# submarine0418/underwater_image_enhancement

Measured on AMD Instinct MI355X. Metric: megapixels/sec enhanced, higher is better.
Workload: dtype f32/f64

## Files before the change

underwater_image_enhancement_amd/csrc/api.hip:

```cpp
#include <cstdarg>
#include <cstdio>
#include <cstring>

#include "common.h"

#include <cstdlib>

namespace uwie {

static thread_local char g_err[512] = "";
static thread_local uwie_ctx *g_ctx = nullptr;
static const Tuning g_default_tuning{};

const Tuning &tune() { return g_ctx ? g_ctx->tune : g_default_tuning; }
uwie_ctx *current_ctx() { return g_ctx; }

void set_error(const char *fmt, ...)
{
    va_list ap;
    va_start(ap, fmt);
    vsnprintf(g_err, sizeof g_err, fmt, ap);
    va_end(ap);
}

// ... 29 lines not shown
        return UWIE_E_HIP;                                                    \
    }

struct KnobName { const char *name; int Tuning::*field; };
const KnobName kKnobs[] = {{"gf_split", &Tuning::gf_split}, {"gf_bands", &Tuning::gf_bands},
                           {"select_generic", &Tuning::select_generic}, {"restore_store", &Tuning::restore_store},
                           {"lin_predict3", &Tuning::lin_predict3}, {"lin_cap", &Tuning::lin_cap},
                           {"lin_no_predict", &Tuning::lin_no_predict}, {"q_hist", &Tuning::q_hist}, {"lin_predict_shift", &Tuning::lin_predict_shift},
                           {"streams", &Tuning::streams}, {"canny_prepass", &Tuning::canny_prepass},
                           {"canny_fault_inject", &Tuning::canny_fault_inject}, {"rank_sweep", &Tuning::rank_sweep},
                           {"gf_fuse", &Tuning::gf_fuse}, {"entry_fuse", &Tuning::entry_fuse}};

void tuning_from_env(Tuning *t)
{
    for (const KnobName &k : kKnobs) {
        char var[64] = "UWIE_";
        size_t n = 5;
        for (const char *c = k.name; *c && n + 1 < sizeof var; ++c) var[n++] = (char)(*c >= 'a' && *c <= 'z' ? *c - 32 : *c);
        var[n] = 0;
        if (const char *e = getenv(var)) t->*(k.field) = atoi(e);
    }
}

bool shape_ok(int B, int H, int W)
{
    if (B < 1 || H < 1 || W < 1) return false;
    const long long npx = (long long)H * W;
    return npx < (1ll << 30) && (long long)B * npx < (1ll << 40);
}

#define UWIE_CHECK_SHAPE(B, H, W) UWIE_REQUIRE(shape_ok(B, H, W), "batch/H/W out of range")
#define UWIE_CHECK_WS(need)                                                                           \
    do {                                                                                              \
        if ((need) > 0 && (!d_workspace || workspace_bytes < (need))) {                               \
            set_error("workspace too small: need %zu bytes, got %zu", (size_t)(need), workspace_bytes); \
            return UWIE_E_WORKSPACE;                                                                  \
        }                                                                                             \
    } while (0)
#define UWIE_TRY(call)            \
    do {                          \
        int _rc = (call);         \
        if (_rc != UWIE_OK) return _rc; \
    } while (0)

struct Pipe {
    int32_t *kind;
    float *A;
    float *pct;
    float *F;
    double *F64;
    double *pct64;
    uint8_t *gray;
    float *t0;
    double *t;
    void *scratch;
    size_t scratch_bytes;
    bool planes;
    uint32_t *qpart;
    int32_t *guess;
};

size_t max5(size_t a, size_t b, size_t c, size_t d, size_t e)
{
    size_t m = a;
    if (b > m) m = b;
    if (c > m) m = c;
    if (d > m) m = d;
    if (e > m) m = e;
    return m;
}

bool dehazes(const uwie_params *p)
{
    if (p->surface == UWIE_SURFACE_SIX) return p->strategy >= 1 && p->strategy <= 3;
    return p->strategy >= UWIE_DICT_STRONG_DEHAZING && p->strategy <= UWIE_DICT_LIGHT_ENHANCEMENT;
}

GuidedRequest u8_guided(const uwie_params *p)
{
    const bool six = p->surface == UWIE_SURFACE_SIX;
    GuidedRequest r{p->gf_ksize, p->gf_eps, p->gf_exact != 0};
    r.fx = six && p->inter_dtype == UWIE_INTER_FX32;
    r.f32_ok = six && p->inter_dtype == UWIE_INTER_F32T && !tune().select_generic;
    r.t0_from_frame = true;
    return r;
}

Pipe carve_pipe(Carver &c, Shape s, const uwie_params *p)
{
    Pipe P{};
    const size_t n = (size_t)s.B * s.npx();
    P.kind = c.take<int32_t>(s.B);
    P.A = c.take<float>((size_t)s.B * 3);
    P.pct = c.take<float>((size_t)s.B * 3 * kMaxPct);
    P.guess = c.take<int32_t>(s.B);
    const bool dz = !p || dehazes(p);
    const bool dict_dz = p && p->surface == UWIE_SURFACE_DICT && dz;
    if (dict_dz) {
        P.F64 = c.take<double>(n * 3);
        P.pct64 = c.take<double>((size_t)s.B * 3 * kMaxPct);
    } else if (!p || (p->surface == UWIE_SURFACE_SIX && dz && (p->strategy == 3 || tune().restore_store || tune().select_generic))) {
        P.F = c.take<float>(n * 3);
    }
    const int tx = p ? p->tiles_x : 8, ty = p ? p->tiles_y : 8;
    const bool gf_planes = dz && (!p || plan_guided(s, u8_guided(p)).planes);
    if (dz) {
        P.gray = c.take<uint8_t>(n);
        if (gf_planes) P.t0 = c.take<float>(n);
        P.t = c.take<double>(n);
    }
    P.scratch_bytes = max5(cast_ws_bytes(s), dz ? airlight_ws_bytes(s) : 0, gf_planes ? guided_ws_bytes(s) : 0,
                           select_ws_bytes(s), clahe_ws_bytes(s, tx > 0 ? tx : 8, ty > 0 ? ty : 8));
    const size_t cw = codes_ws_bytes(s, tx > 0 ? tx : 8, ty > 0 ? ty : 8);
    if (cw > P.scratch_bytes) P.scratch_bytes = cw;
    if (dz && !gf_planes && P.scratch_bytes < n * sizeof(float)) P.scratch_bytes = n * sizeof(float);
    size_t qoff = 0;
    if (dz && p && p->surface == UWIE_SURFACE_SIX && p->cast_correct && p->forced_cast < 0 && entry_fuse_takes(s, p->min_size)) {
        qoff = (std::max(cast_ws_bytes(s), airlight_ws_bytes(s)) + 255) & ~size_t(255);
        if (P.scratch_bytes < qoff + quad_part_bytes(s)) P.scratch_bytes = qoff + quad_part_bytes(s);
    }
    P.scratch = c.take<char>(P.scratch_bytes);
    P.planes = gf_planes;
    if (dz && !gf_planes) P.t0 = static_cast<float *>(P.scratch);
    if (qoff && P.scratch) P.qpart = reinterpret_cast<uint32_t *>(static_cast<char *>(P.scratch) + qoff);
    return P;
}

uwie_params merged_params(const uwie_params *ps, int n, Shape s)
{
    uwie_params m = ps[0];
    m.surface = UWIE_SURFACE_SIX;
    m.strategy = 2;
    for (int i = 0; i < n; ++i) {
        if (ps[i].surface == UWIE_SURFACE_SIX && ps[i].strategy == 3) m.strategy = 3;
        if (ps[i].tiles_x > m.tiles_x) m.tiles_x = ps[i].tiles_x;
        if (ps[i].tiles_y > m.tiles_y) m.tiles_y = ps[i].tiles_y;
        if (ps[i].surface == UWIE_SURFACE_SIX && ps[i].strategy <= 3 && plan_guided(s, u8_guided(&ps[i])).planes) m.gf_exact = 1;
    }
    return m;
}

int stage_guided(const Pipe &P, Shape s, const uwie_params *p, const FuseT0Args &frame, hipStream_t st, int *t_is_f32 = nullptr)
{
    const GuidedPlan g = plan_guided(s, u8_guided(p));
    UWIE_REQUIRE(!g.planes || (P.planes && P.t0 != P.scratch), "guided filter: the workspace layout has no planes for the exact-order filter");
    if (g.t0) UWIE_TRY(launch_trans_init(frame.rgb, frame.kind, frame.A, s, frame.omega, frame.norm_eps, frame.pre_clip, P.t0, st));
    UWIE_TRY(launch_guided_plan(g, s, P.gray, P.t0, P.t, P.scratch, st, &frame));
    if (t_is_f32) *t_is_f32 = g.t_f32;
    return UWIE_OK;
}

int stretch_f32(const float *img, float *out, Shape s, double lo, double hi, float eps, float *pct, void *ws, hipStream_t st)
{
    const double q[2] = {lo, hi};
    UWIE_TRY(launch_percentiles(img, 0, s, q, 2, pct, ws, st));
    return launch_stretch_apply_f32(img, pct, 2, 0, 1, eps, out, s, st);
}

bool quad_from_cast(const uwie_params *p, const Pipe &P) { return P.qpart && p->forced_cast < 0 && p->cast_correct; }

int six_cast(uwie_ctx *ctx, const uint8_t *d_in, Shape s, const uwie_params *p, const Pipe &P, const int32_t **kind,
             hipStream_t st, bool then_airlight = false)
{
    *kind = nullptr;
    if (p->forced_cast >= 0) {
        UWIE_TRY(launch_set_kind(P.kind, s.B, p->forced_cast, st));
        *kind = P.kind;
    } else if (p->cast_correct) {
        const EntryFuse ef{P.qpart, tune().entry_fuse == 2 ? nullptr : P.gray, P.guess, p->gray_shift};
        UWIE_TRY(launch_cast_classify(ctx, d_in, s, P.kind, nullptr, P.scratch, st, then_airlight && quad_from_cast(p, P) ? &ef : nullptr));
        *kind = P.kind;
    }
    return UWIE_OK;
}

int six_airlight(uwie_ctx *ctx, const uint8_t *d_in, const int32_t *kind, Shape s, const uwie_params *p, const Pipe &P,
                 hipStream_t st, bool after_cast = false)
{
    const bool fused = after_cast && quad_from_cast(p, P);
    return launch_airlight(ctx, d_in, kind, P.gray, s, p->min_size, P.A, nullptr, P.scratch, st,
                           fused && tune().entry_fuse != 2 ? 0 : p->gray_shift, fused ? P.qpart : nullptr);
}

int six_dehaze_tail(uwie_ctx *ctx, const uint8_t *d_in, const int32_t *kind, Shape s, const uwie_params *p, const Pipe &P,
                    uint8_t *d_out_u8, float *d_out_f32, hipStream_t st)
{
    const float eps = 1e-6f;
    const int k = p->strategy;
    int t_is_f32 = 0;
    UWIE_TRY(stage_guided(P, s, p, FuseT0Args{d_in, kind, P.A, (float)p->omega, 1e-6f, 1}, st, &t_is_f32));
    SelectPlan plan;
    const double q[4] = {p->L_low, p->L_high, p->wb_percentile, 100 - p->wb_percentile};
    const RestoreSrc src{d_in, kind, P.A, P.t, t_is_f32};
    bool recompute = false;
    if (tune().select_generic) {
        UWIE_TRY(select_begin<float>(s, q, k == 3 ? 4 : 2, P.scratch, st, &plan));
        UWIE_TRY(launch_restore_planar_hist(d_in, kind, P.A, P.t, s, P.F, plan.ghist, st, false, nullptr, t_is_f32));
        UWIE_TRY(select_run(plan, P.F, 1, s, true, st));
    } else {
        recompute = k != 3 && !tune().restore_store;
// ... 1503 lines not shown
```

underwater_image_enhancement_amd/csrc/common.h:

```cpp
#pragma once
#include <hip/hip_runtime.h>
#include <stddef.h>
#include <stdint.h>

#include "../../include/uwie.h"

namespace uwie {

void set_error(const char *fmt, ...);
#define UWIE_HIP_CHECK(expr)                                                            \
    do {                                                                                \
        hipError_t _e = (expr);                                                         \
        if (_e != hipSuccess) {                                                         \
            ::uwie::set_error("%s failed: %s (%s:%d)", #expr, hipGetErrorString(_e), __FILE__, __LINE__); \
            return UWIE_E_HIP;                                                          \
        }                                                                               \
    } while (0)
#define UWIE_LAUNCH_CHECK() UWIE_HIP_CHECK(hipGetLastError())
#define UWIE_REQUIRE(cond, msg)                 \
    do {                                        \
        if (!(cond)) {                          \
            ::uwie::set_error("%s", msg);       \
            return UWIE_E_INVALID;              \
        }                                       \
// ... 159 lines not shown
uint32_t *canny_strong_flags(void *ws, Shape s);
int launch_make_full_regions(Region *d_regions, Shape s, hipStream_t st);

int launch_region_stats(const uint8_t *d_in, const int32_t *d_kind, const Region *d_regs, int nreg, int max_rows,
                        int max_cols, Shape s, float *csum, int maxChunks, float *tot, float *mean, float *vtot,
                        hipStream_t st);
int launch_frame_hist(const uint8_t *d_in, Shape s, uint32_t *d_hist, hipStream_t st);
size_t features_ws_bytes(Shape s);
int launch_features_u8(const uint8_t *d_in, Shape s, float *d_out, void *ws, hipStream_t st);

size_t quality_ws_bytes(Shape s);
int launch_quality_scores(uwie_ctx *ctx, const uint8_t *d_u8, const float *d_f32, Shape s, int gray_shift,
                          const double *weights8, double *d_scores, void *ws, hipStream_t st);

bool feature_extractor_has_dct(int H, int W);
int feature_extractor_count(int H, int W);
size_t feature_extractor_ws_bytes(Shape s);
int launch_feature_extractor(uwie_ctx *ctx, const uint8_t *d_u8, const float *d_f32, Shape s, int gray_shift, double *d_out,
                             void *ws, hipStream_t st);

int launch_resize_rgb(const uwie_frame_desc *d_desc, int B, int oh, int ow, const uint8_t *d_flips, uint8_t *d_u8, float *d_f32,
                      float *d_norm, const float *mean3, const float *std3, uint32_t *d_status, hipStream_t st);

struct ClsNode {
    double thr;
    int32_t left, right, feat, miss;
};
struct ClsModel {
    int kind, F, C, T, K, S;
    double lr, gamma;
    const double *mean, *scale;
    const int32_t *tree_off;
    const ClsNode *nodes;
    const double *value;
    const double *init;
    const double *svT;
    const double *coef;
    const double *rho;
    const double *prob_a, *prob_b;
    const int32_t *sv_start;
};
int classify_model_check(const uwie_model_desc *d);
size_t classify_blob_bytes(const uwie_model_desc *d);
ClsModel classify_pack(const uwie_model_desc *d, void *host_blob, const void *dev_blob);
int launch_classify(const ClsModel &m, const double *d_rows, int B, int32_t *d_label, double *d_proba, uint32_t *d_status,
                    hipStream_t st);

int launch_pick_best(const double *d_scores, int n, Shape s, const uint8_t *d_all, int32_t *d_best, uint8_t *d_out, hipStream_t st);

size_t guided_ws_bytes(Shape s);
size_t box_ws_bytes(Shape s);
int launch_trans_init(const uint8_t *d_in, const int32_t *d_kind, const float *d_A, Shape s, float omega, float norm_eps,
                      int pre_clip, float *d_t0, hipStream_t st);
int launch_box_filter_f64(const double *d_src, double *d_dst, Shape s, int k, void *ws, hipStream_t st);
int launch_guided(const uint8_t *d_gray, const float *d_t0, Shape s, int k, double eps, double *d_t, void *ws,
                  hipStream_t st);
int launch_guided_p64(const uint8_t *d_gray, const double *d_t0, Shape s, int k, double eps, double *d_t, void *ws, hipStream_t st);

enum GuidedRoute {
    GF_EXACT,
    GF_FAST,
    GF_PIPE,
    GF_SPLIT,
    GF_FUSED,
};
struct GuidedRequest {
    int k;
    double eps;
    bool exact = false;
    bool fx = false;
    bool f32_ok = false;
    bool t0_from_frame = false;
    bool t0_f64 = false;
};
struct GuidedPlan {
    GuidedRoute route;
    int k;
    double eps;
    bool t_f32;
    bool ring_fx;
    bool t0_f64;
    bool t0;
    bool planes;
    int TH;
    int iy0, band, nb, rows;
    int pipe_bands;
};
GuidedPlan plan_guided(Shape s, const GuidedRequest &r);
struct FuseT0Args {
    const uint8_t *rgb;
    const int32_t *kind;
    const float *A;
    float omega, norm_eps;
    int pre_clip;
};
int launch_guided_plan(const GuidedPlan &g, Shape s, const uint8_t *d_gray, const void *d_t0, double *d_t, void *ws, hipStream_t st,
                       const FuseT0Args *frame = nullptr);
int guided_fast_th(Shape s, int k);
int launch_guided_fast(const uint8_t *d_gray, const float *d_t0, Shape s, int k, int TH, double eps, double *d_t, hipStream_t st);

constexpr int kMaxPct = 4;
size_t select_ws_bytes(Shape s);
template <typename V>
int launch_percentiles(const V *d_vals, int planar, Shape s, const double *q_percent, int nq, V *d_out, void *ws, hipStream_t st);
int launch_widen_f32(const float *d_in, double *d_out, size_t n, hipStream_t st);

constexpr int kSelGroupStride = 2 * kMaxPct * 2048;
constexpr int kSelOsStride = 2 * kMaxPct;
struct LinState;
struct SelectPlan {
    void *state;
    uint32_t *ghist;
    void *os;
    double t[kMaxPct];
    int nq;
    bool is64;
    LinState *lin;
    void *lists;
    uint32_t *flags;
    uint32_t cap;
    bool predicted;
    uint32_t ranks[2 * kMaxPct];
    template <typename V>
    V *lists_as() const { return static_cast<V *>(lists); }
};
constexpr int kLinBins = 2050;
__host__ __device__ inline uint32_t lin_digit(float x)
{
    if (!(x > 0.0f)) return 0;
    if (x >= 1.0f) return kLinBins - 1;
    const uint32_t d = (uint32_t)(x * 2048.0f);
    return 1 + (d > 2047u ? 2047u : d);
}
__host__ __device__ inline uint32_t lin_digit(double x)
{
    if (!(x > 0.0)) return 0;
    if (x >= 1.0) return kLinBins - 1;
    const uint32_t d = (uint32_t)(x * 2048.0);
    return 1 + (d > 2047u ? 2047u : d);
}
constexpr int kLinLists = 2 * kMaxPct;
constexpr uint32_t kLinNoWin = 0x80000000u;
struct LinState {
    uint32_t rr[2 * kMaxPct];
    uint32_t qbin[2 * kMaxPct];
    uint32_t gid[2 * kMaxPct];
    uint32_t gbin[2 * kMaxPct];
// ... 130 lines not shown
```

underwater_image_enhancement_amd/csrc/k_guided.hip:

```cpp
#include "common.h"
#include "devutil.h"
#include "guided_wave.h"

namespace uwie {

namespace {

typedef double2 __attribute__((aligned(8))) gdouble2_a8;
typedef float4 __attribute__((aligned(4))) gfloat4_a4;
typedef uint32_t __attribute__((aligned(1))) gu32_a1;
typedef double gd2v __attribute__((ext_vector_type(2), aligned(8)));
__device__ __forceinline__ void st_d2(double *p, double v0, double v1) { __builtin_nontemporal_store(gd2v{v0, v1}, reinterpret_cast<gd2v *>(p)); }
__device__ __forceinline__ void st_d1(double *p, double v) { __builtin_nontemporal_store(v, p); }
__device__ __forceinline__ double ld_d1(const double *p) { return __builtin_nontemporal_load(p); }

struct SrcPlanes1 {
    const double *p;
    int H, W;
    static constexpr const char *kName = "k_box_rows_lane<SrcPlanes1>";
    static constexpr int NP = 1;
    static constexpr int CH = 16;
    struct Raw {
        double v;
    };
// ... 631 lines not shown
    const uint8_t *img = in + (size_t)b * npx * 3;
    const bool aligned = (npx & 3) == 0;
    for (int i = threadIdx.x; i < 768; i += 256) {
        const int c = i >> 8;
        nrm[c][i & 255] = px_val(i & 255, px_atten(k, c)) / (A[b * 3 + c] + norm_eps);
    }
    __syncthreads();
    float *trow = t0 + (size_t)b * npx;
    auto t_of = [&](const Px4 &v, int i) {
        const float dark = fminf(fminf(nrm[0][v.r[i]], nrm[1][v.g[i]]), nrm[2][v.b[i]]);
        float t = 1.0f - omega * dark;
        if (pre_clip) t = fminf(fmaxf(t, 0.1f), 1.0f);
        return t;
    };
#ifndef UWIE_TI_PREFETCH
#define UWIE_TI_PREFETCH 1
#endif
    if (UWIE_TI_PREFETCH && aligned && npx >= 4) {
        const int stride = gridDim.x * 1024, plast = npx - 4;
        int p = (blockIdx.x * 256 + threadIdx.x) * 4;
        auto ld3 = [&](int q) { return *reinterpret_cast<const uint3 *>(img + (size_t)q * 3); };
        uint3 nx = ld3(min(p, plast));
        for (; p < npx; p += stride) {
            const uint3 w = nx;
            nx = ld3(min(p + stride, plast));
            Px4 v;
            v.r[0] = w.x & 255; v.g[0] = (w.x >> 8) & 255; v.b[0] = (w.x >> 16) & 255;
            v.r[1] = w.x >> 24; v.g[1] = w.y & 255; v.b[1] = (w.y >> 8) & 255;
            v.r[2] = (w.y >> 16) & 255; v.g[2] = w.y >> 24; v.b[2] = w.z & 255;
            v.r[3] = (w.z >> 8) & 255; v.g[3] = (w.z >> 16) & 255; v.b[3] = w.z >> 24;
            *reinterpret_cast<float4 *>(trow + p) = make_float4(t_of(v, 0), t_of(v, 1), t_of(v, 2), t_of(v, 3));
        }
        return;
    }
    for (int p = (blockIdx.x * 256 + threadIdx.x) * 4; p < npx; p += gridDim.x * 1024) {
        const int n = min(4, npx - p);
        const Px4 v = load_px4(img + (size_t)p * 3, n, aligned);
        float o[4];
#pragma unroll
        for (int i = 0; i < 4; ++i) {
            const float dark = fminf(fminf(nrm[0][v.r[i]], nrm[1][v.g[i]]), nrm[2][v.b[i]]);
            float t = 1.0f - omega * dark;
            if (pre_clip) t = fminf(fmaxf(t, 0.1f), 1.0f);
            o[i] = t;
        }
        if (aligned && n == 4) {
            *reinterpret_cast<float4 *>(trow + p) = make_float4(o[0], o[1], o[2], o[3]);
        } else {
            for (int i = 0; i < n; ++i) trow[p + i] = o[i];
        }
    }
}

}

int launch_trans_init(const uint8_t *d_in, const int32_t *d_kind, const float *d_A, Shape s, float omega, float norm_eps,
                      int pre_clip, float *d_t0, hipStream_t st)
{
#ifndef UWIE_TI_BLOCKS
#define UWIE_TI_BLOCKS 16384
#endif
    int blocks = grid_for((s.npx() + 3) / 4, 4096);
    {
        int want = cdiv(UWIE_TI_BLOCKS, s.B);
        want = want < 32 ? 32 : want;
        if (blocks > want) blocks = want;
    }
    UWIE_LAUNCH(k_trans_init, dim3(blocks, s.B), dim3(256), 0, st, d_in, d_kind, d_A, (int)s.npx(), omega,
                       norm_eps, pre_clip, d_t0);
    UWIE_LAUNCH_CHECK();
    return UWIE_OK;
}

size_t box_ws_bytes(Shape s)
{
    Carver c(nullptr);
    c.take<double>((size_t)s.B * s.npx());
    return c.total();
}

int launch_box_filter_f64(const double *d_src, double *d_dst, Shape s, int k, void *ws, hipStream_t st)
{
    Carver c(ws);
    const size_t n = (size_t)s.B * s.npx();
    double *rs = c.take<double>(n);
    launch_rows_planes(d_src, nullptr, s, rs, n, k, st);
    UWIE_LAUNCH_CHECK();
    launch_cols(rs, n, EpiStore1{d_dst}, s, k, st);
    UWIE_LAUNCH_CHECK();
    return UWIE_OK;
}

size_t guided_ws_bytes(Shape s)
{
    Carver c(nullptr);
    c.take<double>((size_t)s.B * s.npx() * 6);
    return c.total();
}

template <class TP>
static int launch_guided_t(const uint8_t *d_gray, const TP *d_t0, Shape s, int k, double eps, double *d_t, void *ws, hipStream_t st)
{
    Carver c(ws);
    const size_t n = (size_t)s.B * s.npx();
    double *rs = c.take<double>(n * 6);
    double *pa = rs + 4 * n, *pb = rs + 5 * n;
// ... 34 lines not shown
```

underwater_image_enhancement_amd/csrc/k_guided_pipe.hip:

```cpp
#include "common.h"
#include "devutil.h"
#include "guided_wave.h"

#include <algorithm>
#include <cmath>
#include <type_traits>
#include <utility>

namespace uwie {

namespace {

#define UWIE_TRY_RC(call)               \
    do {                                \
        const int _rc = (call);         \
        if (_rc != UWIE_OK) return _rc; \
    } while (0)

#ifndef UWIE_GF_MINBAND
#define UWIE_GF_MINBAND 32
#endif
constexpr int kPipeSlots = 128;
struct PipeGeom {
    int H, W, band;
// ... 493 lines not shown
        } else rest.template swap_at<S - 1>(a0, a1, gg);
    }
    template <int S>
    __device__ __forceinline__ void set_at(uint32_t a0, uint32_t a1, uint32_t gg)
    {
        if constexpr (S == 0) {
            t0 = a0; t1 = a1;
            if constexpr (G) g = gg;
        } else rest.template set_at<S - 1>(a0, a1, gg);
    }
};
template <bool G>
struct RawRing<0, G> {
    template <int S> __device__ __forceinline__ void swap_at(uint32_t &, uint32_t &, uint32_t &) {}
    template <int S> __device__ __forceinline__ void set_at(uint32_t, uint32_t, uint32_t) {}
};

#ifndef SPLIT_QUAD
#define SPLIT_QUAD 1
#endif
#ifndef SPLIT_MUL24
#define SPLIT_MUL24 1
#endif
__device__ __forceinline__ double dpp_next(double v)
{
    const int lo = __builtin_amdgcn_update_dpp(0, __double2loint(v), 0x130, 0xf, 0xf, true);
    const int hi = __builtin_amdgcn_update_dpp(0, __double2hiint(v), 0x130, 0xf, 0xf, true);
    return __hiloint2double(hi, lo);
}
__device__ __forceinline__ uint32_t dpp_next(uint32_t v)
{
    return (uint32_t)__builtin_amdgcn_update_dpp(0, (int)v, 0x130, 0xf, 0xf, true);
}
__device__ __forceinline__ double2 q_add(double2 a, double2 b) { return make_double2(a.x + b.x, a.y + b.y); }
__device__ __forceinline__ double2 q_sub(double2 a, double2 b) { return make_double2(a.x - b.x, a.y - b.y); }
__device__ __forceinline__ double2 q_next(double2 v) { return make_double2(dpp_next(v.x), dpp_next(v.y)); }
__device__ __forceinline__ uint2 q_add(uint2 a, uint2 b) { return make_uint2(a.x + b.x, a.y + b.y); }
__device__ __forceinline__ uint2 q_sub(uint2 a, uint2 b) { return make_uint2(a.x - b.x, a.y - b.y); }
__device__ __forceinline__ uint2 q_next(uint2 v) { return make_uint2(dpp_next(v.x), dpp_next(v.y)); }

template <int K>
struct SplitCfg {
    static constexpr bool RAWREG = K <= 16;
    static constexpr int NB = K % 3 == 0 ? 3 : K > 16 ? 2 : K % 5 == 0 ? 5 : 2;
    static constexpr int AR = K > 16 ? 3 : 0;
    static constexpr bool STAGE_FIRST = AR > 0;
    static constexpr int pad_bytes = 16 * (PipeCfg<K>::M + 1) > 128 ? 16 * (PipeCfg<K>::M + 1) : 128;
    static constexpr int s2_bytes = STAGE_FIRST ? 2048 : 2048 + pad_bytes;
    static constexpr int ring_lds_bytes = (K - AR) * (PipeCfg<K>::NL + 1) * 16;
    static_assert(!STAGE_FIRST || ring_lds_bytes >= pad_bytes, "the look-ahead must stay inside the allocation");
    static constexpr int lds_bytes = ring_lds_bytes + PipeCfg<K>::s1_doubles * 8 + s2_bytes;
};

__device__ __forceinline__ uint32_t fuse_t0_bits(const float *tab, uint32_t r, uint32_t g, uint32_t b, float omega, int pre_clip)
{
    const float dark = fminf(fminf(tab[r], tab[256 + g]), tab[512 + b]);
    float t = __fsub_rn(1.0f, __fmul_rn(omega, dark));
    if (pre_clip) t = fminf(fmaxf(t, 0.1f), 1.0f);
    return __float_as_uint(t);
}

template <int K, bool EDGE, typename TOut, bool FUSE = false>
__device__ __forceinline__ void split_body(const uint8_t *__restrict__ gray, const float *__restrict__ t0, TOut *__restrict__ tout,
                                           const SplitGeom &g, const PipeConsts &cs, char *lds, int3 bid, int lane_in = -1,
                                           const float *tab = nullptr, float omega = 0.0f, int pre_clip = 0)
{
    using C = PipeCfg<K>;
    constexpr int a = C::a, Lb = C::Lb, NV = C::NV, RC = K, NL = C::NL, M = C::M, SW = C::SW;
    constexpr int NB = SplitCfg<K>::NB;
    static_assert(RC % NB == 0, "the ring period must be a multiple of the row buffers");
    constexpr bool RAWREG = SplitCfg<K>::RAWREG;
    constexpr int NLp = NL + 1, EB = 16;
    constexpr int AR = SplitCfg<K>::AR;
    constexpr int ring_bytes = SplitCfg<K>::ring_lds_bytes;
    constexpr uint32_t stage_base = SplitCfg<K>::STAGE_FIRST ? 0u : (uint32_t)ring_bytes;
    constexpr uint32_t ring_base = SplitCfg<K>::STAGE_FIRST ? 3072u + 2048u : 0u;
    constexpr double K2 = (double)(K * K);
    const int lane = lane_in >= 0 ? lane_in : (int)threadIdx.x;
    const int H = g.H, W = g.W;
    const int x_lo = bid.x * NV;
    const int y_lo = g.y0 + bid.y * g.band;
    const int r_lo = y_lo - a;
    const size_t img = (size_t)bid.z * H * W;
    const uint32_t npx = (uint32_t)H * (uint32_t)W;
    constexpr uint32_t kTB = FUSE ? 3u : 4u;
    const __amdgpu_buffer_rsrc_t rT = FUSE ? pipe_rsrc(reinterpret_cast<const uint8_t *>(t0) + img * 3, npx * 3u) : pipe_rsrc(t0 + img, npx * 4u),
                                 rG = pipe_rsrc(gray + img, npx), rO = pipe_rsrc(tout + img, npx * (uint32_t)sizeof(TOut));
    const uint32_t pitch_t = (uint32_t)W * kTB, pitch_g = (uint32_t)W, pitch_o = (uint32_t)W * (uint32_t)sizeof(TOut);

    const int xo0 = x_lo + 2 * lane;
    int craw[2], fix_addr[2];
    bool fix_need[2], fix_odd[2];
    uint32_t ofs_t[2], ofs_g[2], ofs_o[2], ofs_q[2];
#pragma unroll
    for (int j = 0; j < 2; ++j) {
        const int sl = 2 * lane + j;
        craw[j] = EDGE ? pipe_reflect(x_lo - 2 * a + sl, W) : x_lo - 2 * a + sl;
        ofs_t[j] = (uint32_t)craw[j] * kTB;
        ofs_g[j] = (uint32_t)craw[j];
        ofs_o[j] = EDGE ? (uint32_t)min(xo0 + j, W - 1) : (uint32_t)min(xo0, W - 2);
        ofs_q[j] = sl < NV && xo0 + j < W ? (uint32_t)(xo0 + j) * (uint32_t)sizeof(TOut) : kNoStore;
        const int c = x_lo - a + sl, cr = pipe_reflect(c, W);
        const int sp = min(max(cr - (x_lo - a), 0), kPipeSlots - 1);
        fix_need[j] = EDGE && cr != c;
        fix_addr[j] = (sp >> 1) << 2;
        fix_odd[j] = sp & 1;
    }

    const uint32_t a_ring = pipe_opaque(ring_base + (uint32_t)min(lane, NLp - 1) * (uint32_t)EB);

#ifndef SPLIT_RAW_G
#define SPLIT_RAW_G 1
#endif
    constexpr bool RAWG = SPLIT_RAW_G && RAWREG && K == 15 && !FUSE;
    struct In {
        uint32_t te[2];
        uint32_t ge[2], go[2];
        uint32_t gl[2];
        uint32_t tl[2];
    };
    auto byte_of = [](const uint32_t (&v)[2], int c) { return EDGE ? v[c] : (c == 0 ? (v[0] & 255u) : (v[0] >> 8)); };
    static_assert(!FUSE || RAWREG, "the fused transmission keeps its rows in the register ring (no leaving-row reload)");
    auto load_rows = [&](uint32_t oe_t, uint32_t oe_g, uint32_t ol_t, uint32_t ol_g, uint32_t oo_g, In &in) {
        if constexpr (!RAWREG) {
            if constexpr (!EDGE) {
                const u32x2 tl = __builtin_amdgcn_raw_buffer_load_b64(rT, ofs_t[0], ol_t, 0);
                in.tl[0] = tl.x; in.tl[1] = tl.y;
            } else {
                in.tl[0] = (uint32_t)__builtin_amdgcn_raw_buffer_load_b32(rT, ofs_t[0], ol_t, 0);
                in.tl[1] = (uint32_t)__builtin_amdgcn_raw_buffer_load_b32(rT, ofs_t[1], ol_t, 0);
            }
        }
        if constexpr (!RAWG) {
            if constexpr (!EDGE) in.gl[0] = (uint16_t)__builtin_amdgcn_raw_buffer_load_b16(rG, ofs_g[0], ol_g, 0);
            else {
                in.gl[0] = (uint8_t)__builtin_amdgcn_raw_buffer_load_b8(rG, ofs_g[0], ol_g, 0);
                in.gl[1] = (uint8_t)__builtin_amdgcn_raw_buffer_load_b8(rG, ofs_g[1], ol_g, 0);
            }
        }
        if constexpr (!EDGE) {
            if constexpr (FUSE) {
                in.te[0] = (uint32_t)__builtin_amdgcn_raw_buffer_load_b32(rT, ofs_t[0], oe_t, 0);
                in.te[1] = (uint16_t)__builtin_amdgcn_raw_buffer_load_b16(rT, ofs_t[0] + 4u, oe_t, 0);
            } else {
                const u32x2 te = __builtin_amdgcn_raw_buffer_load_b64(rT, ofs_t[0], oe_t, 0);
                in.te[0] = te.x; in.te[1] = te.y;
            }
            in.ge[0] = (uint16_t)__builtin_amdgcn_raw_buffer_load_b16(rG, ofs_g[0], oe_g, 0);
            in.go[0] = (uint16_t)__builtin_amdgcn_raw_buffer_load_b16(rG, ofs_o[0], oo_g, 0);
            in.ge[1] = in.go[1] = 0;
        } else {
#pragma unroll
            for (int j = 0; j < 2; ++j) {
                if constexpr (FUSE) {
                    const uint32_t r = (uint8_t)__builtin_amdgcn_raw_buffer_load_b8(rT, ofs_t[j], oe_t, 0);
                    const uint32_t gg = (uint8_t)__builtin_amdgcn_raw_buffer_load_b8(rT, ofs_t[j] + 1u, oe_t, 0);
                    const uint32_t bb = (uint8_t)__builtin_amdgcn_raw_buffer_load_b8(rT, ofs_t[j] + 2u, oe_t, 0);
                    in.te[j] = r | (gg << 8) | (bb << 16);
                } else {
                    in.te[j] = (uint32_t)__builtin_amdgcn_raw_buffer_load_b32(rT, ofs_t[j], oe_t, 0);
                }
                in.ge[j] = (uint8_t)__builtin_amdgcn_raw_buffer_load_b8(rG, ofs_g[j], oe_g, 0);
                in.go[j] = (uint8_t)__builtin_amdgcn_raw_buffer_load_b8(rG, ofs_o[j], oo_g, 0);
            }
        }
    };
    auto te_bits = [&](const In &in, uint32_t (&tb)[2]) {
        if constexpr (!FUSE) {
            tb[0] = in.te[0]; tb[1] = in.te[1];
        } else if constexpr (!EDGE) {
            const uint32_t w0 = in.te[0], w1 = in.te[1];
            tb[0] = fuse_t0_bits(tab, w0 & 255u, (w0 >> 8) & 255u, (w0 >> 16) & 255u, omega, pre_clip);
            tb[1] = fuse_t0_bits(tab, w0 >> 24, w1 & 255u, (w1 >> 8) & 255u, omega, pre_clip);
        } else {
#pragma unroll
            for (int j = 0; j < 2; ++j)
                tb[j] = fuse_t0_bits(tab, in.te[j] & 255u, (in.te[j] >> 8) & 255u, (in.te[j] >> 16) & 255u, omega, pre_clip);
        }
    };

    double V1p[2] = {0.0, 0.0}, V1gp[2] = {0.0, 0.0};
    uint32_t Sg[2] = {0, 0}, Sgg[2] = {0, 0};
    double V2a[2] = {0.0, 0.0}, V2b[2] = {0.0, 0.0};
    RawRing<RAWREG ? RC : 0, RAWG> raw;
    auto prologue_row = [&](auto j_tag) {
        constexpr int J = decltype(j_tag)::value;
        const uint32_t row = (uint32_t)pipe_reflect(r_lo - a + J, H);
        uint32_t tb[2], gq[2];
#pragma unroll
        for (int c = 0; c < 2; ++c) {
            gq[c] = (uint8_t)__builtin_amdgcn_raw_buffer_load_b8(rG, ofs_g[c], row * pitch_g, 0);
            if constexpr (FUSE) {
                const uint32_t r = (uint8_t)__builtin_amdgcn_raw_buffer_load_b8(rT, ofs_t[c], row * pitch_t, 0);
                const uint32_t gg = (uint8_t)__builtin_amdgcn_raw_buffer_load_b8(rT, ofs_t[c] + 1u, row * pitch_t, 0);
                const uint32_t bb = (uint8_t)__builtin_amdgcn_raw_buffer_load_b8(rT, ofs_t[c] + 2u, row * pitch_t, 0);
                tb[c] = fuse_t0_bits(tab, r, gg, bb, omega, pre_clip);
            } else {
                tb[c] = (uint32_t)__builtin_amdgcn_raw_buffer_load_b32(rT, ofs_t[c], row * pitch_t, 0);
            }
            const double p = (double)__uint_as_float(tb[c]);
            Sg[c] += gq[c];
            Sgg[c] += gq[c] * gq[c];
            V1p[c] += p;
            V1gp[c] += (double)gq[c] * p;
        }
        if constexpr (RAWREG) raw.template set_at<J>(tb[0], tb[1], gq[0] | (gq[1] << 8));
    };
    [&]<int... J>(std::integer_sequence<int, J...>) { (prologue_row(IC<J>{}), ...); }(std::make_integer_sequence<int, RC>{});
    RegRing<RC> rb;
    rb.clear();
#pragma unroll
    for (int s = 0; s < RC - AR; ++s) *reinterpret_cast<double2 *>(lds + a_ring + (uint32_t)(s * NLp * EB)) = make_double2(0.0, 0.0);
    RegRing<AR> ra;
    ra.clear();

    const uint32_t a16 = pipe_opaque(stage_base + (uint32_t)lane * 16u);
    const uint32_t a8 = pipe_opaque(stage_base + 2048u + (uint32_t)lane * 8u);
    const double2 *pp1 = reinterpret_cast<const double2 *>(lds + a16), *vv1 = pp1 + SW;
    const uint2 *pi = reinterpret_cast<const uint2 *>(lds + a8), *vi = pi + SW;
    const double2 *pp2 = reinterpret_cast<const double2 *>(lds + a16 + 3072u), *vv2 = pp2 + SW;
    static_assert(C::s1_doubles * 8 == 3072 && (SplitCfg<K>::STAGE_FIRST || SplitCfg<K>::s2_bytes >= 2048 + 16 * (C::M + 1)), "staging layout");
    auto window2 = [&](const double2 *pp, const double2 *vv, double2 P, double2 v1, double2 (&o)[2]) {
        double2 m0 = pp[1], m1 = pp[2];
#pragma unroll
        for (int d = 3; d < M; d += 2) { const double2 t = pp[d]; m0.x += t.x; m0.y += t.y; }
#pragma unroll
        for (int d = 4; d < M; d += 2) { const double2 t = pp[d]; m1.x += t.x; m1.y += t.y; }
        const double2 f0 = vv[M];
        const double midx = m0.x + m1.x, midy = m0.y + m1.y;
        if constexpr (K & 1) {
            const double2 pm = pp[M];
            o[0] = make_double2((P.x + midx) + f0.x, (P.y + midy) + f0.y);
            o[1] = make_double2((v1.x + midx) + pm.x, (v1.y + midy) + pm.y);
        } else {
            o[0] = make_double2(P.x + midx, P.y + midy);
            o[1] = make_double2((v1.x + midx) + f0.x, (v1.y + midy) + f0.y);
        }
    };
    constexpr bool QUAD = SPLIT_QUAD != 0 && ((K & 1) || !(M & 1));
    static_assert(!QUAD || !(K & 1) || (M & 1), "odd windows: an odd number of pair sums on either side of the lane's own");
    double2 keep1 = make_double2(0.0, 0.0), keep2 = keep1;
    uint2 keepI = make_uint2(0u, 0u);
    auto stage_q = [&](auto *line, auto s0, auto s1, auto &keep) {
        const auto P = q_add(s0, s1);
        const auto Pn = q_next(P);
        const auto R = q_add(P, Pn);
        line[0] = R;
        if constexpr (K & 1) {
            line[SW] = s1;
// ... 163 lines not shown
    int gr = i0 - Lb - 2;
    int yo = y_lo;
    auto issue = [&](In &fill) {
        asm volatile("" : "+s"(re), "+s"(gr), "+s"(yo));
        const uint32_t er = (uint32_t)pipe_reflect(re, H), lr = (uint32_t)pipe_reflect(re - RC, H);
        const uint32_t og = (uint32_t)min(max(gr, 0), H - 1);
        load_rows(er * pitch_t, er * pitch_g, lr * pitch_t, lr * pitch_g, og * pitch_g, fill);
        ++re;
        ++gr;
    };
    In buf[NB];
    [&]<int... Q>(std::integer_sequence<int, Q...>) { (issue(buf[Q]), ...); }(std::make_integer_sequence<int, NB - 1>{});
    auto one = [&](auto warm_tag, auto slot_tag, In &fill, const In &use) {
        issue(fill);
        step(warm_tag, slot_tag, use, (uint32_t)yo * pitch_o, yo < H);
        if constexpr (!decltype(warm_tag)::value) ++yo;
        __builtin_amdgcn_sched_barrier(0);
    };
    auto period = [&](auto warm_tag) {
        auto at = [&](auto slot_tag) {
            constexpr int S = decltype(slot_tag)::value;
            one(warm_tag, slot_tag, buf[(S + NB - 1) % NB], buf[S % NB]);
        };
        [&]<int... Q>(std::integer_sequence<int, Q...>) { (at(IC<Q>{}), ...); }(std::make_integer_sequence<int, RC>{});
    };
    period(std::true_type{});
    const int nper = (((int)bid.y == g.nbands - 1 ? g.y_end - y_lo : g.band) + RC - 1) / RC;
    for (int p = 0; p < nper; ++p) period(std::false_type{});
}


template <int K, typename TOut>
__global__ void __launch_bounds__(64) __attribute__((amdgpu_waves_per_eu(2, 2)))
k_guided_split(const uint8_t *__restrict__ gray, const float *__restrict__ t0, TOut *__restrict__ tout, SplitGeom g, PipeConsts cs)
{
    extern __shared__ double2 lds_raw[];
    char *lds = reinterpret_cast<char *>(lds_raw);
    int3 bid = {(int)blockIdx.x, (int)blockIdx.y, (int)blockIdx.z};
    if (g.xcd_fold) {
        const uint32_t gx = gridDim.x, gy = gridDim.y, n = gx * gy * gridDim.z;
        const uint32_t lin = blockIdx.x + gx * (blockIdx.y + gy * blockIdx.z);
        const uint32_t xcd = lin & 7u, idx = lin >> 3, q = n >> 3, r = n & 7u;
        const uint32_t log = (xcd < r ? xcd * (q + 1) : r * (q + 1) + (xcd - r) * q) + idx;
        bid.x = (int)(log % gx);
        bid.y = (int)((log / gx) % gy);
        bid.z = (int)(log / (gx * gy));
    }
    const int x_lo = bid.x * PipeCfg<K>::NV;
    const bool edge = x_lo - 2 * PipeCfg<K>::a < 0 || x_lo - 2 * PipeCfg<K>::a + kPipeSlots > g.W;
    if (edge) split_body<K, true, TOut>(gray, t0, tout, g, cs, lds, bid);
    else split_body<K, false, TOut>(gray, t0, tout, g, cs, lds, bid);
}

template <int K, typename TOut>
__global__ void __launch_bounds__(512) __attribute__((amdgpu_waves_per_eu(2, 2)))
k_guided_split8(const uint8_t *__restrict__ gray, FuseT0Args fz, TOut *__restrict__ tout, SplitGeom g, PipeConsts cs, int nstrips)
{
    extern __shared__ double2 lds_raw[];
    char *lds = reinterpret_cast<char *>(lds_raw);
    constexpr int per_wave = SplitCfg<K>::lds_bytes;
    float *tab = reinterpret_cast<float *>(lds + 8 * per_wave);
    const int wave = __builtin_amdgcn_readfirstlane((int)(threadIdx.x >> 6)), lane = threadIdx.x & 63;
    int grp = (int)blockIdx.x, b = (int)blockIdx.z;
    if (g.xcd_fold) {
        const uint32_t gx = gridDim.x, n = gx * gridDim.z, lin = blockIdx.x + gx * blockIdx.z;
        const uint32_t xcd = lin & 7u, idx = lin >> 3, q = n >> 3, r = n & 7u;
        const uint32_t log = (xcd < r ? xcd * (q + 1) : r * (q + 1) + (xcd - r) * q) + idx;
        grp = (int)(log % gx);
        b = (int)(log / gx);
    }
    {
        const int kd = fz.kind ? fz.kind[b] : 0;
        for (int i = threadIdx.x; i < 768; i += 512) {
            const int c = i >> 8;
            tab[i] = px_val(i & 255, px_atten(kd, c)) / (fz.A[b * 3 + c] + fz.norm_eps);
        }
    }
    __syncthreads();
    const int item = grp * 8 + wave;
    if (item >= nstrips * g.nbands) return;
    const int3 bid = {item % nstrips, item / nstrips, b};
    const int x_lo = bid.x * PipeCfg<K>::NV;
    const bool edge = x_lo - 2 * PipeCfg<K>::a < 0 || x_lo - 2 * PipeCfg<K>::a + kPipeSlots > g.W;
    const float *t0 = reinterpret_cast<const float *>(fz.rgb);
    if (edge) split_body<K, true, TOut, true>(gray, t0, tout, g, cs, lds + wave * per_wave, bid, lane, tab, fz.omega, fz.pre_clip);
    else split_body<K, false, TOut, true>(gray, t0, tout, g, cs, lds + wave * per_wave, bid, lane, tab, fz.omega, fz.pre_clip);
}

template <int K, typename TOut>
int launch_split8(const uint8_t *d_gray, const FuseT0Args &fz, Shape s, const PipeConsts &cs, TOut *d_t, int y0, int band, int nbands,
                  int y_end, hipStream_t st)
{
    using C = PipeCfg<K>;
    constexpr int lds = 8 * SplitCfg<K>::lds_bytes + 768 * 4;
    static_assert(lds <= 160 * 1024, "eight strips and the table have to fit one CU");
#ifndef UWIE_SPLIT8_FOLD
#define UWIE_SPLIT8_FOLD 1
#endif
    SplitGeom g{s.H, s.W, y0, band, y_end, UWIE_SPLIT8_FOLD, nbands};
    const int nstrips = cdiv(s.W, C::NV);
    uwie_ctx *ctx = current_ctx();
    const int bit = std::is_same<TOut, double>::value ? 1 : 2;
    if (ctx && !(ctx->attr_gf_split8 & bit)) {
        UWIE_HIP_CHECK(hipFuncSetAttribute(reinterpret_cast<const void *>(&k_guided_split8<K, TOut>),
                                           hipFuncAttributeMaxDynamicSharedMemorySize, lds));
        ctx->attr_gf_split8 |= bit;
    }
    {
        UWIE_PROF("k_guided_split8", st);
        hipLaunchKernelGGL((k_guided_split8<K, TOut>), dim3(cdiv((long long)nstrips * nbands, 8), 1, s.B), dim3(512), (size_t)lds, st, d_gray,
                           fz, d_t, g, cs, nstrips);
    }
    UWIE_LAUNCH_CHECK();
    return UWIE_OK;
}

template <int K, typename TOut>
int launch_split(const uint8_t *d_gray, const float *d_t0, Shape s, const PipeConsts &cs, TOut *d_t, int y0, int band, int nbands,
                 int y_end, hipStream_t st)
{
    using C = PipeCfg<K>;
    constexpr int lds = SplitCfg<K>::lds_bytes;
#ifndef UWIE_SPLIT_FOLD
#define UWIE_SPLIT_FOLD 1
#endif
    SplitGeom g{s.H, s.W, y0, band, y_end, UWIE_SPLIT_FOLD, nbands};
    const int nstrips = cdiv(s.W, C::NV);
    {
        UWIE_PROF("k_guided_split", st);
        hipLaunchKernelGGL((k_guided_split<K, TOut>), dim3(nstrips, nbands, s.B), dim3(64), (size_t)lds, st, d_gray, d_t0, d_t, g, cs);
    }
    UWIE_LAUNCH_CHECK();
    return UWIE_OK;
}

template <int K, bool FX, typename TOut>
int launch_pipe(const uint8_t *d_gray, const float *d_t0, Shape s, const PipeConsts &cs, TOut *d_t, int nbands, hipStream_t st,
                const int *border = nullptr)
{
    using C = PipeCfg<K>;
    constexpr int lds = C::lds_bytes(FX);
    const int nstrips = cdiv(s.W, C::NV);
    PipeGeom g{};
    g.H = s.H; g.W = s.W;
    g.band = cdiv(s.H, nbands);
    int gy = cdiv(s.H, g.band);
    if (border) {
        g.iy0 = border[0]; g.iy1 = border[1]; g.iband = border[2];
        gy = 2 + border[3];
        g.is0 = border[4]; g.is1 = border[5];
    }
    {
        UWIE_PROF("k_guided_pipe", st);
        hipLaunchKernelGGL((k_guided_pipe<K, FX, TOut>), dim3(nstrips, gy, s.B), dim3(64), (size_t)lds, st, d_gray, d_t0, d_t, g, cs);
    }
    UWIE_LAUNCH_CHECK();
    return UWIE_OK;
}

int pipe_bands(Shape s, int k, bool fx, int forced)
{
    const int lds = k == 10 ? PipeCfg<10>::lds_bytes(fx) : k == 15 ? PipeCfg<15>::lds_bytes(fx) : PipeCfg<20>::lds_bytes(fx);
    const int resident = 256 * std::max(1, std::min(8, (160 * 1024) / lds));
// ... 88 lines not shown
int launch_wave(const GuidedPlan &g, const uint8_t *d_gray, const float *d_t0, Shape s, TOut *d_t, hipStream_t st)
{
    const PipeConsts cs = pipe_consts(g);
    if (g.k == 10) return launch_pipe_plan<10>(g, d_gray, d_t0, s, cs, d_t, st);
    if (g.k == 15) return launch_pipe_plan<15>(g, d_gray, d_t0, s, cs, d_t, st);
    return launch_pipe_plan<20>(g, d_gray, d_t0, s, cs, d_t, st);
}

}

GuidedPlan plan_guided(Shape s, const GuidedRequest &r)
{
    GuidedPlan g{};
    g.k = r.k;
    g.eps = r.eps;
    g.t0 = true;
    const bool free_order = !r.exact && !r.t0_f64 && r.k >= 1 && r.k <= 1024;
    const bool wave = free_order && (r.k == 10 || r.k == 15 || r.k == 20) && s.W >= 2 * r.k && s.H >= 4 * r.k && s.B <= 65535 &&
                      r.eps > 0.0;
    if (!wave) {
        g.TH = free_order ? guided_fast_th(s, r.k) : 0;
        g.route = g.TH ? GF_FAST : GF_EXACT;
        g.t0_f64 = r.t0_f64;
        g.planes = !g.TH;
        return g;
    }
    const Tuning &tu = tune();
    int Sa, Sb;
    g.ring_fx = r.fx && fx_scales(r.eps, &Sa, &Sb);
    g.t_f32 = r.f32_ok && !g.ring_fx && !(s.W & 1);
    g.pipe_bands = pipe_bands(s, r.k, g.ring_fx, tu.gf_bands);
    g.route = GF_PIPE;
    if (!g.ring_fx && tu.gf_split && split_plan(s, r.k, tu.gf_bands, &g.iy0, &g.band, &g.nb, &g.rows)) {
        g.route = GF_SPLIT;
        if (r.k == 15 && r.t0_from_frame && !r.fx && tu.gf_fuse) {
            g.route = GF_FUSED;
            g.t0 = false;
        }
    }
    return g;
}

int launch_guided_plan(const GuidedPlan &g, Shape s, const uint8_t *d_gray, const void *d_t0, double *d_t, void *ws, hipStream_t st,
                       const FuseT0Args *frame)
{
    const float *t0 = static_cast<const float *>(d_t0);
    switch (g.route) {
    case GF_EXACT:
        UWIE_REQUIRE(ws, "guided filter: the exact-order kernels need the workspace's planes");
        if (g.t0_f64) return launch_guided_p64(d_gray, static_cast<const double *>(d_t0), s, g.k, g.eps, d_t, ws, st);
        return launch_guided(d_gray, t0, s, g.k, g.eps, d_t, ws, st);
    case GF_FAST: return launch_guided_fast(d_gray, t0, s, g.k, g.TH, g.eps, d_t, st);
    case GF_FUSED:
        UWIE_REQUIRE(frame, "guided filter: the fused plan computes t0 from the frame");
        if (g.t_f32) return launch_split8<15, float>(d_gray, *frame, s, pipe_consts(g), reinterpret_cast<float *>(d_t), g.iy0, g.band, g.nb, s.H, st);
        return launch_split8<15, double>(d_gray, *frame, s, pipe_consts(g), d_t, g.iy0, g.band, g.nb, s.H, st);
    default:
        if (g.t_f32) return launch_wave(g, d_gray, t0, s, reinterpret_cast<float *>(d_t), st);
        return launch_wave(g, d_gray, t0, s, d_t, st);
    }
}

}
```

Baseline: 57650.

## Precompute per-image transmission table and shrink fused guided-filter workgroups

```diff
diff --git a/underwater_image_enhancement_amd/csrc/api.hip b/underwater_image_enhancement_amd/csrc/api.hip
--- a/underwater_image_enhancement_amd/csrc/api.hip
+++ b/underwater_image_enhancement_amd/csrc/api.hip
@@ -105,6 +105,7 @@
     double *pct64;
     uint8_t *gray;
     float *t0;
+    float *ttab;
     double *t;
     void *scratch;
     size_t scratch_bytes;
@@ -135,7 +136,7 @@
     GuidedRequest r{p->gf_ksize, p->gf_eps, p->gf_exact != 0};
     r.fx = six && p->inter_dtype == UWIE_INTER_FX32;
     r.f32_ok = six && p->inter_dtype == UWIE_INTER_F32T && !tune().select_generic;
-    r.t0_from_frame = true;
+    r.t0_from_frame = p->omega >= 0.0;
     return r;
 }
 
@@ -167,6 +168,7 @@
     const size_t cw = codes_ws_bytes(s, tx > 0 ? tx : 8, ty > 0 ? ty : 8);
     if (cw > P.scratch_bytes) P.scratch_bytes = cw;
     if (dz && !gf_planes && P.scratch_bytes < n * sizeof(float)) P.scratch_bytes = n * sizeof(float);
+    if (dz && P.scratch_bytes < (size_t)s.B * 768 * sizeof(float)) P.scratch_bytes = (size_t)s.B * 768 * sizeof(float);
     size_t qoff = 0;
     if (dz && p && p->surface == UWIE_SURFACE_SIX && p->cast_correct && p->forced_cast < 0 && entry_fuse_takes(s, p->min_size)) {
         qoff = (std::max(cast_ws_bytes(s), airlight_ws_bytes(s)) + 255) & ~size_t(255);
@@ -175,6 +177,7 @@
     P.scratch = c.take<char>(P.scratch_bytes);
     P.planes = gf_planes;
     if (dz && !gf_planes) P.t0 = static_cast<float *>(P.scratch);
+    if (dz) P.ttab = static_cast<float *>(P.scratch);
     if (qoff && P.scratch) P.qpart = reinterpret_cast<uint32_t *>(static_cast<char *>(P.scratch) + qoff);
     return P;
 }
@@ -197,8 +200,11 @@
 {
     const GuidedPlan g = plan_guided(s, u8_guided(p));
     UWIE_REQUIRE(!g.planes || (P.planes && P.t0 != P.scratch), "guided filter: the workspace layout has no planes for the exact-order filter");
+    FuseT0Args fz = frame;
+    fz.tab = P.ttab;
     if (g.t0) UWIE_TRY(launch_trans_init(frame.rgb, frame.kind, frame.A, s, frame.omega, frame.norm_eps, frame.pre_clip, P.t0, st));
-    UWIE_TRY(launch_guided_plan(g, s, P.gray, P.t0, P.t, P.scratch, st, &frame));
+    else UWIE_TRY(launch_trans_table(frame.kind, frame.A, s.B, frame.omega, frame.norm_eps, frame.pre_clip, P.ttab, st));
+    UWIE_TRY(launch_guided_plan(g, s, P.gray, P.t0, P.t, P.scratch, st, &fz));
     if (t_is_f32) *t_is_f32 = g.t_f32;
     return UWIE_OK;
 }
diff --git a/underwater_image_enhancement_amd/csrc/common.h b/underwater_image_enhancement_amd/csrc/common.h
--- a/underwater_image_enhancement_amd/csrc/common.h
+++ b/underwater_image_enhancement_amd/csrc/common.h
@@ -235,6 +235,8 @@
 size_t box_ws_bytes(Shape s);
 int launch_trans_init(const uint8_t *d_in, const int32_t *d_kind, const float *d_A, Shape s, float omega, float norm_eps,
                       int pre_clip, float *d_t0, hipStream_t st);
+int launch_trans_table(const int32_t *d_kind, const float *d_A, int B, float omega, float norm_eps, int pre_clip, float *d_tab,
+                       hipStream_t st);
 int launch_box_filter_f64(const double *d_src, double *d_dst, Shape s, int k, void *ws, hipStream_t st);
 int launch_guided(const uint8_t *d_gray, const float *d_t0, Shape s, int k, double eps, double *d_t, void *ws,
                   hipStream_t st);
@@ -276,6 +278,7 @@
     const float *A;
     float omega, norm_eps;
     int pre_clip;
+    const float *tab;
 };
 int launch_guided_plan(const GuidedPlan &g, Shape s, const uint8_t *d_gray, const void *d_t0, double *d_t, void *ws, hipStream_t st,
                        const FuseT0Args *frame = nullptr);
diff --git a/underwater_image_enhancement_amd/csrc/k_guided.hip b/underwater_image_enhancement_amd/csrc/k_guided.hip
--- a/underwater_image_enhancement_amd/csrc/k_guided.hip
+++ b/underwater_image_enhancement_amd/csrc/k_guided.hip
@@ -707,6 +707,28 @@
     }
 }
 
+__global__ void __launch_bounds__(256) k_trans_table(const int32_t *__restrict__ kind, const float *__restrict__ A, float omega,
+                                                     float norm_eps, int pre_clip, float *__restrict__ tab)
+{
+    const int b = blockIdx.x;
+    const int k = kind ? kind[b] : 0;
+    for (int i = threadIdx.x; i < 768; i += 256) {
+        const int c = i >> 8;
+        const float q = px_val(i & 255, px_atten(k, c)) / (A[b * 3 + c] + norm_eps);
+        float t = __fsub_rn(1.0f, __fmul_rn(omega, q));
+        if (pre_clip) t = fminf(fmaxf(t, 0.1f), 1.0f);
+        tab[(size_t)b * 768 + i] = t;
+    }
+}
+
+}
+
+int launch_trans_table(const int32_t *d_kind, const float *d_A, int B, float omega, float norm_eps, int pre_clip, float *d_tab,
+                       hipStream_t st)
+{
+    UWIE_LAUNCH(k_trans_table, dim3(B), dim3(256), 0, st, d_kind, d_A, omega, norm_eps, pre_clip, d_tab);
+    UWIE_LAUNCH_CHECK();
+    return UWIE_OK;
 }
 
 int launch_trans_init(const uint8_t *d_in, const int32_t *d_kind, const float *d_A, Shape s, float omega, float norm_eps,
diff --git a/underwater_image_enhancement_amd/csrc/k_guided_pipe.hip b/underwater_image_enhancement_amd/csrc/k_guided_pipe.hip
--- a/underwater_image_enhancement_amd/csrc/k_guided_pipe.hip
+++ b/underwater_image_enhancement_amd/csrc/k_guided_pipe.hip
@@ -569,18 +569,15 @@
     static constexpr int lds_bytes = ring_lds_bytes + PipeCfg<K>::s1_doubles * 8 + s2_bytes;
 };
 
-__device__ __forceinline__ uint32_t fuse_t0_bits(const float *tab, uint32_t r, uint32_t g, uint32_t b, float omega, int pre_clip)
-{
-    const float dark = fminf(fminf(tab[r], tab[256 + g]), tab[512 + b]);
-    float t = __fsub_rn(1.0f, __fmul_rn(omega, dark));
-    if (pre_clip) t = fminf(fmaxf(t, 0.1f), 1.0f);
-    return __float_as_uint(t);
+__device__ __forceinline__ uint32_t fuse_t0_bits(const float *tab, uint32_t r, uint32_t g, uint32_t b)
+{
+    return __float_as_uint(fmaxf(fmaxf(tab[r], tab[256 + g]), tab[512 + b]));
 }
 
 template <int K, bool EDGE, typename TOut, bool FUSE = false>
 __device__ __forceinline__ void split_body(const uint8_t *__restrict__ gray, const float *__restrict__ t0, TOut *__restrict__ tout,
                                            const SplitGeom &g, const PipeConsts &cs, char *lds, int3 bid, int lane_in = -1,
-                                           const float *tab = nullptr, float omega = 0.0f, int pre_clip = 0)
+                                           const float *tab = nullptr)
 {
     using C = PipeCfg<K>;
     constexpr int a = C::a, Lb = C::Lb, NV = C::NV, RC = K, NL = C::NL, M = C::M, SW = C::SW;
@@ -687,12 +684,12 @@
             tb[0] = in.te[0]; tb[1] = in.te[1];
         } else if constexpr (!EDGE) {
             const uint32_t w0 = in.te[0], w1 = in.te[1];
-            tb[0] = fuse_t0_bits(tab, w0 & 255u, (w0 >> 8) & 255u, (w0 >> 16) & 255u, omega, pre_clip);
-            tb[1] = fuse_t0_bits(tab, w0 >> 24, w1 & 255u, (w1 >> 8) & 255u, omega, pre_clip);
+            tb[0] = fuse_t0_bits(tab, w0 & 255u, (w0 >> 8) & 255u, (w0 >> 16) & 255u);
+            tb[1] = fuse_t0_bits(tab, w0 >> 24, w1 & 255u, (w1 >> 8) & 255u);
         } else {
 #pragma unroll
             for (int j = 0; j < 2; ++j)
-                tb[j] = fuse_t0_bits(tab, in.te[j] & 255u, (in.te[j] >> 8) & 255u, (in.te[j] >> 16) & 255u, omega, pre_clip);
+                tb[j] = fuse_t0_bits(tab, in.te[j] & 255u, (in.te[j] >> 8) & 255u, (in.te[j] >> 16) & 255u);
         }
     };
 
@@ -711,7 +708,7 @@
                 const uint32_t r = (uint8_t)__builtin_amdgcn_raw_buffer_load_b8(rT, ofs_t[c], row * pitch_t, 0);
                 const uint32_t gg = (uint8_t)__builtin_amdgcn_raw_buffer_load_b8(rT, ofs_t[c] + 1u, row * pitch_t, 0);
                 const uint32_t bb = (uint8_t)__builtin_amdgcn_raw_buffer_load_b8(rT, ofs_t[c] + 2u, row * pitch_t, 0);
-                tb[c] = fuse_t0_bits(tab, r, gg, bb, omega, pre_clip);
+                tb[c] = fuse_t0_bits(tab, r, gg, bb);
             } else {
                 tb[c] = (uint32_t)__builtin_amdgcn_raw_buffer_load_b32(rT, ofs_t[c], row * pitch_t, 0);
             }
@@ -981,14 +978,20 @@
     else split_body<K, false, TOut>(gray, t0, tout, g, cs, lds, bid);
 }
 
+#ifndef UWIE_SPLIT8_WAVES
+#define UWIE_SPLIT8_WAVES 4
+#endif
+constexpr int kSplit8Waves = UWIE_SPLIT8_WAVES;
+static_assert(kSplit8Waves >= 3 && kSplit8Waves <= 8, "three wavefronts copy the table; a CU holds eight strips");
 template <int K, typename TOut>
-__global__ void __launch_bounds__(512) __attribute__((amdgpu_waves_per_eu(2, 2)))
+__global__ void __launch_bounds__(64 * kSplit8Waves) __attribute__((amdgpu_waves_per_eu(2, 2)))
 k_guided_split8(const uint8_t *__restrict__ gray, FuseT0Args fz, TOut *__restrict__ tout, SplitGeom g, PipeConsts cs, int nstrips)
 {
     extern __shared__ double2 lds_raw[];
     char *lds = reinterpret_cast<char *>(lds_raw);
     constexpr int per_wave = SplitCfg<K>::lds_bytes;
-    float *tab = reinterpret_cast<float *>(lds + 8 * per_wave);
+    static_assert(per_wave % 16 == 0, "the table behind the wavefronts' regions is copied in 16-byte pieces");
+    float *tab = reinterpret_cast<float *>(lds + kSplit8Waves * per_wave);
     const int wave = __builtin_amdgcn_readfirstlane((int)(threadIdx.x >> 6)), lane = threadIdx.x & 63;
     int grp = (int)blockIdx.x, b = (int)blockIdx.z;
     if (g.xcd_fold) {
@@ -998,22 +1001,16 @@
         grp = (int)(log % gx);
         b = (int)(log / gx);
     }
-    {
-        const int kd = fz.kind ? fz.kind[b] : 0;
-        for (int i = threadIdx.x; i < 768; i += 512) {
-            const int c = i >> 8;
-            tab[i] = px_val(i & 255, px_atten(kd, c)) / (fz.A[b * 3 + c] + fz.norm_eps);
-        }
-    }
+    if (threadIdx.x < 192) reinterpret_cast<float4 *>(tab)[threadIdx.x] = reinterpret_cast<const float4 *>(fz.tab + (size_t)b * 768)[threadIdx.x];
     __syncthreads();
-    const int item = grp * 8 + wave;
+    const int item = grp * kSplit8Waves + wave;
     if (item >= nstrips * g.nbands) return;
     const int3 bid = {item % nstrips, item / nstrips, b};
     const int x_lo = bid.x * PipeCfg<K>::NV;
     const bool edge = x_lo - 2 * PipeCfg<K>::a < 0 || x_lo - 2 * PipeCfg<K>::a + kPipeSlots > g.W;
     const float *t0 = reinterpret_cast<const float *>(fz.rgb);
-    if (edge) split_body<K, true, TOut, true>(gray, t0, tout, g, cs, lds + wave * per_wave, bid, lane, tab, fz.omega, fz.pre_clip);
-    else split_body<K, false, TOut, true>(gray, t0, tout, g, cs, lds + wave * per_wave, bid, lane, tab, fz.omega, fz.pre_clip);
+    if (edge) split_body<K, true, TOut, true>(gray, t0, tout, g, cs, lds + wave * per_wave, bid, lane, tab);
+    else split_body<K, false, TOut, true>(gray, t0, tout, g, cs, lds + wave * per_wave, bid, lane, tab);
 }
 
 template <int K, typename TOut>
@@ -1021,8 +1018,8 @@
                   int y_end, hipStream_t st)
 {
     using C = PipeCfg<K>;
-    constexpr int lds = 8 * SplitCfg<K>::lds_bytes + 768 * 4;
-    static_assert(lds <= 160 * 1024, "eight strips and the table have to fit one CU");
+    constexpr int lds = kSplit8Waves * SplitCfg<K>::lds_bytes + 768 * 4;
+    static_assert((8 / kSplit8Waves) * lds <= 160 * 1024, "a CU's eight strips and their workgroups' tables have to fit its LDS");
 #ifndef UWIE_SPLIT8_FOLD
 #define UWIE_SPLIT8_FOLD 1
 #endif
@@ -1037,7 +1034,7 @@
     }
     {
         UWIE_PROF("k_guided_split8", st);
-        hipLaunchKernelGGL((k_guided_split8<K, TOut>), dim3(cdiv((long long)nstrips * nbands, 8), 1, s.B), dim3(512), (size_t)lds, st, d_gray,
+        hipLaunchKernelGGL((k_guided_split8<K, TOut>), dim3(cdiv((long long)nstrips * nbands, kSplit8Waves), 1, s.B), dim3(64 * kSplit8Waves), (size_t)lds, st, d_gray,
                            fz, d_t, g, cs, nstrips);
     }
     UWIE_LAUNCH_CHECK();
@@ -1232,7 +1229,7 @@
         return launch_guided(d_gray, t0, s, g.k, g.eps, d_t, ws, st);
     case GF_FAST: return launch_guided_fast(d_gray, t0, s, g.k, g.TH, g.eps, d_t, st);
     case GF_FUSED:
-        UWIE_REQUIRE(frame, "guided filter: the fused plan computes t0 from the frame");
+        UWIE_REQUIRE(frame && frame->tab, "guided filter: the fused plan looks t0 up from the frame through its table");
         if (g.t_f32) return launch_split8<15, float>(d_gray, *frame, s, pipe_consts(g), reinterpret_cast<float *>(d_t), g.iy0, g.band, g.nb, s.H, st);
         return launch_split8<15, double>(d_gray, *frame, s, pipe_consts(g), d_t, g.iy0, g.band, g.nb, s.H, st);
     default:
```

After: 56870. -1.4%, worse.
